# facebookresearch/sylph-few-shot-detection

Measured on AMD Instinct MI355X. Metric: query images/sec, R50-FPN 5-way 5-shot 800x1333 (whole job), higher is better.
Workload: dtype bf16

## Files before the change

### sylph-few-shot-detection_amd/csrc/conv_hpipe.hip

```cpp
#include <stdlib.h>

#include "common.h"

#ifndef SYLPH_ABLATE
#undef HP_NOWAITV
#undef HP_NOLDS
#undef HP_NOLOAD
#undef HP_NOEPI
#undef HP_TIMING
#endif

namespace sylph {

typedef __attribute__((address_space(3))) void* lds_ptr_t;
typedef const __attribute__((address_space(1))) void* gbl_ptr_t;

namespace {
constexpr int PNT = 512;
constexpr int BSTAGE = 256 * 64;
constexpr int NSTAGE = 4;
constexpr int HPROWS = 256;
constexpr int HBUF = 2 * HPROWS * 64;
constexpr int HALO_OFF = NSTAGE * BSTAGE;
constexpr int COEF_OFF = HALO_OFF + 2 * HBUF;
constexpr int COEF_MAX_CIN = 512;
constexpr int LDS_BYTES = COEF_OFF + 2 * COEF_MAX_CIN * 8;
constexpr int SCP = 256 + 4;
static_assert(64 * SCP * 4 <= LDS_BYTES, "epilogue tile must fit");

constexpr int NPIECE = 2 * HPROWS / 128;
constexpr int nload(int t) { return ((t % 9 + 9) % 9) < NPIECE ? 3 : 2; }

#define HP_SCHED_FENCE __builtin_amdgcn_sched_barrier(0)
#define HP_BAR()                                   \
  do {                                             \
    asm volatile("" ::: "memory");                 \
    HP_SCHED_FENCE;                                \
    __builtin_amdgcn_s_barrier();                  \
    HP_SCHED_FENCE;                                \
    asm volatile("" ::: "memory");                 \
  } while (0)
#ifdef HP_NOWAITV
#define HP_WAITV(N) asm volatile("" ::: "memory")
#else
#define HP_WAITV(N) asm volatile("s_waitcnt vmcnt(%0)" ::"n"(N) : "memory")
#endif
#define HP_WAITL() asm volatile("s_waitcnt lgkmcnt(0)" ::: "memory")
}

template <bool GNIN>
__global__ __launch_bounds__(PNT, 1) void conv_hpipe_kernel(const ConvArgs a) {
  typedef bf16_t T;
  extern __shared__ __attribute__((aligned(16))) char smem[];

  const int L = blockIdx.x;
  const int xcd = L & 7, q0 = L >> 3;
  const int chunk = (a.n_mtiles + 7) >> 3;
  const int m_local = q0 / a.n_ntiles;
  const int nt = q0 - m_local * a.n_ntiles;
  const int mt = xcd * chunk + m_local;
  if (m_local >= chunk || mt >= a.n_mtiles) return;
#ifdef HP_TIMING
  const unsigned long long hp_t0 = __builtin_readcyclecounter();
  unsigned long long hp_t1 = 0, hp_t2 = 0;
#endif

  const int tid = threadIdx.x, lane = tid & 63;
  const int wave = __builtin_amdgcn_readfirstlane(tid >> 6);
  const int wm = wave >> 2, wn = wave & 3;
  const int l31 = lane & 31, lh = lane >> 5;

  int2 tl0 = a.tiles[2 * mt], tl1 = a.tiles[2 * mt + 1];
  const int rot_key = (int)((unsigned)tl0.x >> 20);
  tl0.x &= 0xfffff;
  const SegDesc sd0 = a.segs[tl0.x], sd1 = a.segs[tl1.x];

  const T* __restrict__ in = reinterpret_cast<const T*>(a.in);
  const T* __restrict__ wt = reinterpret_cast<const T*>(a.wt);
  const T* __restrict__ zero = reinterpret_cast<const T*>(a.zeros);
  const int Cin = a.Cin;
  const int ncc = Cin >> 5;
  const int goff = a.group_cout > 0 ? ((nt * 256) / a.group_cout) * a.group_in_off : 0;
  const int c0 = (rot_key + nt) % ncc;

  const int r4 = tid >> 2, s4 = tid & 3;
  const char* hptr[NPIECE];
  unsigned hmask = 0, hcs = 0;
#pragma unroll
  for (int g = 0; g < NPIECE; ++g) {
    const bool p1 = g >= NPIECE / 2;
    const SegDesc& sd = p1 ? sd1 : sd0;
    const int ty = p1 ? tl1.y : tl0.y;
    const int h = g * 128 + r4 - (p1 ? HPROWS : 0);
    const int PW = sd.pw, HP = sd.hpitch, HR = (sd.ph + 2) * HP;
    const int hy = (int)(((unsigned)h * sd.inv_hw2) >> 16), hx = h - hy * HP;
    const int iy = (ty >> 16) - 1 + hy, ix = (ty & 0xffff) - 1 + hx;
    const bool ok = h < HR && hx < PW + 2 && (unsigned)iy < (unsigned)sd.in_H && (unsigned)ix < (unsigned)sd.in_W;
    const int cs = s4 ^ (((hy * PW + hx) >> 2) & 3);
    hcs |= (unsigned)cs << (2 * g);
    hptr[g] = ok ? reinterpret_cast<const char*>(in + ((size_t)(sd.in_row0 + iy * sd.in_W + ix) * a.in_ld + cs * 8 + goff + c0 * 32))
                 : reinterpret_cast<const char*>(zero + s4 * 8);
    hmask |= (ok ? 1u : 0u) << g;
  }
  const char* const wtile = reinterpret_cast<const char*>(wt) + (size_t)nt * ncc * 9 * BSTAGE;
  const unsigned wvo = (unsigned)tid * 16u;
  bool loads_on = true;
  auto issue_halo = [&](int g, int buf) {
    if (!loads_on) return;
    {
    char* d = smem + HALO_OFF + buf * HBUF + g * 8192 + wave * 1024;
    __builtin_amdgcn_global_load_lds((gbl_ptr_t)hptr[g], (lds_ptr_t)d, 16, 0, 0);
    }
  };
  auto advance_halo = [&](int cc_next) {
    const int step = (c0 + cc_next == ncc) ? (32 - Cin) * 2 : 64;
#pragma unroll
    for (int g = 0; g < NPIECE; ++g) hptr[g] += ((hmask >> g) & 1u) ? step : 0;
  };
  auto issue_w = [&](int stage, int j, int blk) {
    if (!loads_on) return;
    {
    char* d = smem + stage * BSTAGE + j * 8192 + wave * 1024;
    const char* src = wtile + (size_t)blk * BSTAGE + j * 8192 + wvo;
    __builtin_amdgcn_global_load_lds((gbl_ptr_t)src, (lds_ptr_t)d, 16, 0, 0);
    }
  };
  auto rot = [&](int cc) { const int c = c0 + cc; return c >= ncc ? c - ncc : c; };

  constexpr bool gn_in = GNIN;
  const bool gn_relu = a.gn_relu != 0;
  typedef unsigned u32x4 __attribute__((ext_vector_type(4)));
  typedef float f32x4v __attribute__((ext_vector_type(4)));
  const unsigned lds0 = (unsigned)(size_t)(__attribute__((address_space(3))) char*)smem;
  u32x4 gx;
  f32x4v gc0, gc1, gc2, gc3;
  auto gn_addr = [&](int g, int cc_of_piece) { return lds0 + HALO_OFF + (cc_of_piece & 1) * HBUF + g * 8192 + tid * 16; };
  auto gn_read = [&](int g, int cc_of_piece) {
    const unsigned d = gn_addr(g, cc_of_piece);
    const int ch = rot(cc_of_piece) * 32 + (int)((hcs >> (2 * g)) & 3u) * 8;
    const unsigned cf = lds0 + COEF_OFF + ((g >= NPIECE / 2 ? Cin : 0) + ch) * 8;
    asm volatile("ds_read_b128 %0, %1" : "=v"(gx) : "v"(d));
    asm volatile("ds_read_b128 %0, %1" : "=v"(gc0) : "v"(cf));
    asm volatile("ds_read_b128 %0, %1 offset:16" : "=v"(gc1) : "v"(cf));
    asm volatile("ds_read_b128 %0, %1 offset:32" : "=v"(gc2) : "v"(cf));
    asm volatile("ds_read_b128 %0, %1 offset:48" : "=v"(gc3) : "v"(cf));
  };
  auto gn_finish = [&](int g, int cc_of_piece) {
    asm volatile("s_waitcnt lgkmcnt(0)" : "+v"(gx), "+v"(gc0), "+v"(gc1), "+v"(gc2), "+v"(gc3));
    const unsigned live = ((hmask >> g) & 1u) ? 0xffffffffu : 0u;
    const f32x4v cs[4] = {gc0, gc1, gc2, gc3};
    typedef float f32x2v __attribute__((ext_vector_type(2)));
    typedef short s16x2v __attribute__((ext_vector_type(2)));
    typedef __attribute__((ext_vector_type(2))) __bf16 bf16x2;
    u32x4 y;
#pragma unroll
    for (int e = 0; e < 4; ++e) {
      const f32x2v xv = {__uint_as_float(gx[e] << 16), __uint_as_float(gx[e] & 0xffff0000u)};
      const f32x2v av = {cs[e][0], cs[e][1]}, bv = {cs[e][2], cs[e][3]};
      const f32x2v r = __builtin_elementwise_fma(xv, av, bv);
      bf16x2 pk;
      pk[0] = (bf16_t)r[0]; pk[1] = (bf16_t)r[1];
      unsigned u = __builtin_bit_cast(unsigned, pk);
      if (gn_relu) {
        const s16x2v z = {0, 0};
        u = __builtin_bit_cast(unsigned, __builtin_elementwise_max(__builtin_bit_cast(s16x2v, u), z));
      }
      y[e] = u & live;
    }
    asm volatile("ds_write_b128 %0, %1" ::"v"(gn_addr(g, cc_of_piece)), "v"(y) : "memory");
  };
  auto gn_piece = [&](int g, int cc_of_piece) { gn_read(g, cc_of_piece); gn_finish(g, cc_of_piece); };

  const SegDesc& sdm = wm ? sd1 : sd0;
  const int PWm = sdm.pw, HW2m = sdm.hpitch;
  int a0[4];
#pragma unroll
  for (int i = 0; i < 4; ++i) {
    const int m = i * 32 + l31;
    const int my = (int)(((unsigned)m * sdm.inv_pw) >> 16);
    a0[i] = (wm * HPROWS + my * HW2m + (m - my * PWm)) * 64;
  }
  int offB[2];
#pragma unroll
  for (int ks = 0; ks < 2; ++ks) offB[ks] = (wn * 64 + l31) * 64 + (((ks * 2 + lh) ^ ((l31 >> 2) & 3)) << 4);

  f32x16 acc[4][2];
#pragma unroll
  for (int i = 0; i < 4; ++i)
#pragma unroll
    for (int j = 0; j < 2; ++j)
#pragma unroll
      for (int r = 0; r < 16; ++r) acc[i][j][r] = 0.f;
  bf16x8 fa[2][4], fb[2][2];

  auto ldfrag = [&](int cc, int t) {
    const int kh = t / 3, kw = t - 3 * kh;
    const char* bs = smem + ((cc + t) & 3) * BSTAGE;
    const char* hs = smem + HALO_OFF + (cc & 1) * HBUF + (kh * HW2m + kw) * 64;
    const int f = ((l31 + kh * PWm + kw) >> 2) & 3;
#ifdef HP_NOLDS
    if (cc + t > 0) return;
#endif
#pragma unroll
    for (int ks = 0; ks < 2; ++ks) {
      const int so = ((ks * 2 + lh) ^ f) << 4;
#pragma unroll
      for (int j = 0; j < 2; ++j) fb[ks][j] = *reinterpret_cast<const bf16x8*>(bs + offB[ks] + j * 2048);
#pragma unroll
      for (int i = 0; i < 4; ++i) fa[ks][i] = *reinterpret_cast<const bf16x8*>(hs + a0[i] + so);
    }
  };

  auto issue_next = [&](int cc, int t) {
    const int t3 = (t + 3) % 9, cc3 = cc + (t + 3) / 9;
    const int blk = cc3 < ncc ? rot(cc3) * 9 + t3 : 0;
    const int st3 = (cc + t + 3) & 3;
    if (t == 0 && cc + 1 < ncc) advance_halo(cc + 1);
    if (t < NPIECE) issue_halo(t, (cc + 1) & 1);
    issue_w(st3, 0, blk);
    issue_w(st3, 1, blk);
  };
  auto mma = [&](int cc, int t) {
    __builtin_amdgcn_s_setprio(1);
    const bool xf = gn_in && t >= 3 && t < 3 + NPIECE;
    if (xf) {
      gn_read(t - 3, cc + 1);
      HP_SCHED_FENCE;
    }
    int n = 0;
#pragma unroll
    for (int ks = 0; ks < 2; ++ks)
#pragma unroll
      for (int i = 0; i < 4; ++i)
#pragma unroll
        for (int j = 0; j < 2; ++j) {
          acc[i][j] = __builtin_amdgcn_mfma_f32_32x32x16_bf16(fb[ks][j], fa[ks][i], acc[i][j], 0, 0, 0);
          if (xf && n == 3) {
            HP_SCHED_FENCE;
            gn_finish(t - 3, cc + 1);
          }
          ++n;
        }
    if (xf) {
#pragma unroll
      for (int k = 0; k < 12; ++k) {
        __builtin_amdgcn_sched_group_barrier(0x008, 1, 0);
        __builtin_amdgcn_sched_group_barrier(0x002, 4, 0);
      }
    }
    __builtin_amdgcn_s_setprio(0);
  };

  auto frags_ready = [&]() {
    asm volatile("" ::"v"(fa[0][0]), "v"(fa[0][1]), "v"(fa[0][2]), "v"(fa[0][3]), "v"(fa[1][0]), "v"(fa[1][1]), "v"(fa[1][2]),
                 "v"(fa[1][3]), "v"(fb[0][0]), "v"(fb[0][1]), "v"(fb[1][0]), "v"(fb[1][1]));
  };

#pragma unroll
  for (int g = 0; g < NPIECE; ++g) issue_halo(g, 0);
#pragma unroll
  for (int t = 0; t < 3; ++t) {
    issue_w(t, 0, c0 * 9 + t);
    issue_w(t, 1, c0 * 9 + t);
  }
#ifdef HP_NOLOAD
  issue_w(3, 0, c0 * 9 + 3); issue_w(3, 1, c0 * 9 + 3);
  for (int g = 0; g < NPIECE; ++g) issue_halo(g, 1);
  HP_WAITV(0);
  loads_on = false;
#endif
  if (gn_in) {
    for (int idx = tid; idx < Cin; idx += PNT) {
      const int pch = idx >= Cin / 2 ? 1 : 0, ch = (idx - pch * (Cin / 2)) * 2;
      const int seg = pch ? tl1.x : tl0.x;
      const float2 c0v = a.gn_coef[(size_t)seg * a.in_ld + goff + ch], c1v = a.gn_coef[(size_t)seg * a.in_ld + goff + ch + 1];
      *reinterpret_cast<float4*>(smem + COEF_OFF + (pch * Cin + ch) * 8) = make_float4(c0v.x, c1v.x, c0v.y, c1v.y);
    }
  }
  HP_WAITV(4);
  if (gn_in) {
    HP_WAITL();
    HP_BAR();
#pragma unroll
    for (int g = 0; g < NPIECE; ++g) gn_piece(g, 0);
    HP_WAITL();
  }
  HP_BAR();
#ifdef HP_TIMING
  hp_t1 = __builtin_readcyclecounter();
#endif

#define HP_PHASE0(t)                      \
  ldfrag(cc, t);                          \
  HP_SCHED_FENCE;                         \
  issue_next(cc, t);                      \
  HP_WAITL();                             \
  if (GNIN) frags_ready();                \
  HP_BAR();                               \
  mma(cc, t);                             \
  HP_WAITV(nload((t) - 1) + nload(t));    \
  HP_BAR();
#define HP_PHASE1(t)                      \
  ldfrag(cc, t);                          \
  HP_SCHED_FENCE;                         \
  issue_next(cc, t);                      \
  HP_WAITV(nload((t) - 1) + nload(t));    \
  HP_WAITL();                             \
  if (GNIN) frags_ready();                \
  HP_BAR();                               \
  mma(cc, t);                             \
  HP_BAR();

  if (wm == 0) {
    for (int cc = 0; cc < ncc; ++cc) {
      HP_PHASE0(0) HP_PHASE0(1) HP_PHASE0(2) HP_PHASE0(3) HP_PHASE0(4) HP_PHASE0(5) HP_PHASE0(6) HP_PHASE0(7) HP_PHASE0(8)
    }
    HP_BAR();
  } else {
    HP_BAR();
    for (int cc = 0; cc < ncc; ++cc) {
      HP_PHASE1(0) HP_PHASE1(1) HP_PHASE1(2) HP_PHASE1(3) HP_PHASE1(4) HP_PHASE1(5) HP_PHASE1(6) HP_PHASE1(7) HP_PHASE1(8)
    }
  }
  asm volatile("s_waitcnt vmcnt(0)" ::: "memory");
  __syncthreads();
#ifdef HP_TIMING
  hp_t2 = __builtin_readcyclecounter();
#endif

  float* const sC = reinterpret_cast<float*>(smem);
  bf16_t* __restrict__ out = reinterpret_cast<bf16_t*>(a.out);
  const int c8 = tid & 31, rr = tid >> 5;
  const int n0 = nt * 256 + c8 * 8;
  float sc[8], sh[8];
#pragma unroll
  for (int h = 0; h < 2; ++h) {
    const float4 s4v = a.scale ? reinterpret_cast<const float4*>(a.scale + n0)[h] : make_float4(1.f, 1.f, 1.f, 1.f);
    const float4 b4v = a.shift ? reinterpret_cast<const float4*>(a.shift + n0)[h] : make_float4(0.f, 0.f, 0.f, 0.f);
    sc[4 * h] = s4v.x; sc[4 * h + 1] = s4v.y; sc[4 * h + 2] = s4v.z; sc[4 * h + 3] = s4v.w;
    sh[4 * h] = b4v.x; sh[4 * h + 1] = b4v.y; sh[4 * h + 2] = b4v.z; sh[4 * h + 3] = b4v.w;
  }
  const bool relu = a.relu_nch > 0;
#pragma unroll
  for (int pp = 0; pp < 2; ++pp) {
    const SegDesc& sp = pp ? sd1 : sd0;
    const int ty = pp ? tl1.y : tl0.y;
    const int oy0 = ty >> 16, ox0 = ty & 0xffff;
    const int PW = sp.pw, NPOS = sp.ph * sp.pw;
    bf16_t* __restrict__ outn = out + (size_t)sp.out_row0 * a.out_ld + n0;
    float gn_n = 0.f, gn_s1 = 0.f, gn_s2 = 0.f;
    const float gn_pv = sh[0];
#pragma unroll
    for (int hp = 0; hp < 2; ++hp) {
      if (pp + hp > 0) lds_barrier();
      if (wm == pp) {
#pragma unroll
        for (int ii = 0; ii < 2; ++ii)
#pragma unroll
          for (int j = 0; j < 2; ++j)
#pragma unroll
            for (int g = 0; g < 4; ++g) {
              const f32x16& c = acc[2 * hp + ii][j];
              *reinterpret_cast<float4*>(sC + (ii * 32 + l31) * SCP + wn * 64 + j * 32 + 8 * g + 4 * lh) =
                  make_float4(c[4 * g], c[4 * g + 1], c[4 * g + 2], c[4 * g + 3]);
            }
      }
      lds_barrier();
#pragma unroll
      for (int it = 0; it < 4; ++it) {
        const int rl = rr + 16 * it;
        const int m = hp * 64 + rl;
        const int my = (int)(((unsigned)m * sp.inv_pw) >> 16);
        const int oy = oy0 + my, ox = ox0 + (m - my * PW);
        if (m < NPOS && oy < sp.out_H && ox < sp.out_W) {
          float v[8];
          const float4 lo = *reinterpret_cast<const float4*>(sC + rl * SCP + c8 * 8);
          const float4 hi = *reinterpret_cast<const float4*>(sC + rl * SCP + c8 * 8 + 4);
          v[0] = lo.x; v[1] = lo.y; v[2] = lo.z; v[3] = lo.w; v[4] = hi.x; v[5] = hi.y; v[6] = hi.z; v[7] = hi.w;
#pragma unroll
          for (int e = 0; e < 8; ++e) v[e] = v[e] * sc[e] + sh[e];
          if (relu) {
#pragma unroll
            for (int e = 0; e < 8; ++e) v[e] = v[e] > 0.f ? v[e] : 0.f;
          }
          if (a.gn_partial) {
#pragma unroll
            for (int e = 0; e < 8; ++e) { const float d = v[e] - gn_pv; gn_s1 += d; gn_s2 = fmaf(d, d, gn_s2); }
            gn_n += 8.f;
          }
#ifndef HP_NOEPI
          store8<bf16_t>(outn + (size_t)(oy * sp.out_W + ox) * a.out_ld, v);
#else
          if (v[0] == 1234.5f) store8<bf16_t>(outn + (size_t)(oy * sp.out_W + ox) * a.out_ld, v);
#endif
        }
      }
    }
    if (a.gn_partial) {
      gn_n += __shfl_xor(gn_n, 32);
      gn_s1 += __shfl_xor(gn_s1, 32);
      gn_s2 += __shfl_xor(gn_s2, 32);
      lds_barrier();
      float* red = sC;
      if (lane < 32) {
        red[(wave * 32 + c8) * 3 + 0] = gn_n;
        red[(wave * 32 + c8) * 3 + 1] = gn_s1;
        red[(wave * 32 + c8) * 3 + 2] = gn_s2;
      }
      lds_barrier();
      if (tid < 32) {
        float N = 0.f, S1 = 0.f, S2 = 0.f;
#pragma unroll
        for (int w = 0; w < 8; ++w) {
          N += red[(w * 32 + c8) * 3 + 0]; S1 += red[(w * 32 + c8) * 3 + 1]; S2 += red[(w * 32 + c8) * 3 + 2];
        }
        const float inv_n = N > 0.f ? 1.f / N : 0.f;
        const float m2 = S2 - S1 * S1 * inv_n;
        float* gp = a.gn_partial + ((size_t)(2 * mt + pp) * (a.Cout >> 3) + (n0 >> 3)) * 3;
        gp[0] = N; gp[1] = gn_pv + S1 * inv_n; gp[2] = m2 > 0.f ? m2 : 0.f;
      }
    }
  }
#ifdef HP_TIMING
  if (L >= 2048 && L < 2048 + 64 && (tid == 0 || tid == 256)) {
    const unsigned long long t3 = __builtin_readcyclecounter();
    printf("blk %d row %d: prologue %llu  K loop %llu  epilogue %llu cycles\n", L, tid >> 8, hp_t1 - hp_t0, hp_t2 - hp_t1, t3 - hp_t2);
  }
#endif
}

__global__ void hpipe_pack_weights_kernel(const bf16_t* __restrict__ w, bf16_t* __restrict__ out, int Cout, int Cin) {
  const size_t i = (size_t)blockIdx.x * blockDim.x + threadIdx.x;
  const size_t nchunks = (size_t)Cout * 9 * Cin / 8;
  if (i >= nchunks) return;
  const int ncc = Cin >> 5;
  const int s = (int)(i & 3), r = (int)((i >> 2) & 255);
  const size_t blk = i >> 10;
  const int t = (int)(blk % 9), c = (int)((blk / 9) % ncc), nt = (int)(blk / (9 * (size_t)ncc));
  const int chunk = s ^ ((r >> 2) & 3);
  const uint4 v = *reinterpret_cast<const uint4*>(w + ((size_t)(nt * 256 + r) * 9 + t) * Cin + c * 32 + chunk * 8);
  *reinterpret_cast<uint4*>(out + i * 8) = v;
}

int launch_hpipe_pack_weights(const void* w, void* out, int Cout, int Cin, hipStream_t s) {
  const size_t nchunks = (size_t)Cout * 9 * Cin / 8;
  hipLaunchKernelGGL(hpipe_pack_weights_kernel, dim3((unsigned)((nchunks + 255) / 256)), dim3(256), 0, s, (const bf16_t*)w, (bf16_t*)out, Cout, Cin);
  return (int)hipGetLastError();
}

bool conv_hpipe_ok(DType dt, bool out_f32, const ConvArgs& a) {
  if (a.gn_coef && (a.Cin > COEF_MAX_CIN || a.group_cout > 0)) return false;
  return dt == DT_BF16 && !out_f32 && !a.stem && !a.in2 && a.res_mode == 0 && a.mul_nch == 0 && a.KH == 3 && a.KW == 3 &&
         a.stride == 1 && a.pad == 1 && (a.relu_nch == 0 || a.relu_nch >= a.Cout) && a.Cout % 256 == 0 && a.Cin % 32 == 0 &&
         a.Cin >= 32 && a.ss_padded_host && (a.out_ld & 7) == 0 && a.zeros != nullptr;
}

#ifdef SYLPH_ABLATE
int launch_conv_hq(const ConvArgs& a, hipStream_t s);
#endif

int launch_conv_hpipe(const ConvArgs& a, hipStream_t s) {
#if defined(SYLPH_ABLATE) && defined(SYLPH_HQ_PROBE)
  static const int hq = SYLPH_AB_ENV("SYLPH_CONV_HQ", 0);
  if (hq) return launch_conv_hq(a, s);
#endif
  static bool attr_set = false;
  if (!attr_set) {
    if (hipFuncSetAttribute((const void*)conv_hpipe_kernel<false>, hipFuncAttributeMaxDynamicSharedMemorySize, LDS_BYTES) != hipSuccess) return -7;
    if (hipFuncSetAttribute((const void*)conv_hpipe_kernel<true>, hipFuncAttributeMaxDynamicSharedMemorySize, LDS_BYTES) != hipSuccess) return -7;
    attr_set = true;
  }
  const int chunk = (a.n_mtiles + 7) / 8;
  const int grid = 8 * chunk * a.n_ntiles;
  if (a.gn_coef) hipLaunchKernelGGL(conv_hpipe_kernel<true>, dim3(grid), dim3(PNT), LDS_BYTES, s, a);
  else hipLaunchKernelGGL(conv_hpipe_kernel<false>, dim3(grid), dim3(PNT), LDS_BYTES, s, a);
  return (int)hipGetLastError();
}

}
```

Before: 2245.

## Switch hpipe conv to 16x16x32 MFMA tiles with new LDS swizzle

Replaces the 32x32x16 bf16 MFMA tiling (4x2 accumulators, two k-substeps) with 16x16x32 MFMA over an 8x4 accumulator grid, and changes the LDS XOR swizzle for halo, weights and the packing kernel to match the new fragment read pattern. The GN input path now converts to bf16 with a vector convert and applies a branch-free max against a floor value instead of a conditional ReLU. The scheduling barriers and epilogue stores are reworked for the new accumulator shape. This trades the larger MFMA for more instructions, each with a shorter latency, and an altered bank-conflict profile.

Measured after the change: 2347 (median of 6 runs). 1.05x the previous value.

```diff
diff --git a/sylph-few-shot-detection_amd/csrc/conv_hpipe.hip b/sylph-few-shot-detection_amd/csrc/conv_hpipe.hip
--- a/sylph-few-shot-detection_amd/csrc/conv_hpipe.hip
+++ b/sylph-few-shot-detection_amd/csrc/conv_hpipe.hip
@@ -68,7 +68,7 @@
   const int tid = threadIdx.x, lane = tid & 63;
   const int wave = __builtin_amdgcn_readfirstlane(tid >> 6);
   const int wm = wave >> 2, wn = wave & 3;
-  const int l31 = lane & 31, lh = lane >> 5;
+  const int l15 = lane & 15, lq = lane >> 4;
 
   int2 tl0 = a.tiles[2 * mt], tl1 = a.tiles[2 * mt + 1];
   const int rot_key = (int)((unsigned)tl0.x >> 20);
@@ -96,7 +96,7 @@
     const int hy = (int)(((unsigned)h * sd.inv_hw2) >> 16), hx = h - hy * HP;
     const int iy = (ty >> 16) - 1 + hy, ix = (ty & 0xffff) - 1 + hx;
     const bool ok = h < HR && hx < PW + 2 && (unsigned)iy < (unsigned)sd.in_H && (unsigned)ix < (unsigned)sd.in_W;
-    const int cs = s4 ^ (((hy * PW + hx) >> 2) & 3);
+    const int cs = s4 ^ ((((hy * PW + hx) >> 2) & 1) << 1);
     hcs |= (unsigned)cs << (2 * g);
     hptr[g] = ok ? reinterpret_cast<const char*>(in + ((size_t)(sd.in_row0 + iy * sd.in_W + ix) * a.in_ld + cs * 8 + goff + c0 * 32))
                  : reinterpret_cast<const char*>(zero + s4 * 8);
@@ -128,7 +128,7 @@
   auto rot = [&](int cc) { const int c = c0 + cc; return c >= ncc ? c - ncc : c; };
 
   constexpr bool gn_in = GNIN;
-  const bool gn_relu = a.gn_relu != 0;
+  const short gn_floor = a.gn_relu != 0 ? (short)0 : (short)-32768;
   typedef unsigned u32x4 __attribute__((ext_vector_type(4)));
   typedef float f32x4v __attribute__((ext_vector_type(4)));
   const unsigned lds0 = (unsigned)(size_t)(__attribute__((address_space(3))) char*)smem;
@@ -158,13 +158,9 @@
       const f32x2v xv = {__uint_as_float(gx[e] << 16), __uint_as_float(gx[e] & 0xffff0000u)};
       const f32x2v av = {cs[e][0], cs[e][1]}, bv = {cs[e][2], cs[e][3]};
       const f32x2v r = __builtin_elementwise_fma(xv, av, bv);
-      bf16x2 pk;
-      pk[0] = (bf16_t)r[0]; pk[1] = (bf16_t)r[1];
-      unsigned u = __builtin_bit_cast(unsigned, pk);
-      if (gn_relu) {
-        const s16x2v z = {0, 0};
-        u = __builtin_bit_cast(unsigned, __builtin_elementwise_max(__builtin_bit_cast(s16x2v, u), z));
-      }
+      const bf16x2 pk = __builtin_convertvector(r, bf16x2);
+      const s16x2v fl = {gn_floor, gn_floor};
+      const unsigned u = __builtin_bit_cast(unsigned, __builtin_elementwise_max(__builtin_bit_cast(s16x2v, pk), fl));
       y[e] = u & live;
     }
     asm volatile("ds_write_b128 %0, %1" ::"v"(gn_addr(g, cc_of_piece)), "v"(y) : "memory");
@@ -173,42 +169,38 @@
 
   const SegDesc& sdm = wm ? sd1 : sd0;
   const int PWm = sdm.pw, HW2m = sdm.hpitch;
-  int a0[4];
-#pragma unroll
-  for (int i = 0; i < 4; ++i) {
-    const int m = i * 32 + l31;
+  int a0[8];
+#pragma unroll
+  for (int i = 0; i < 8; ++i) {
+    const int m = i * 16 + l15;
     const int my = (int)(((unsigned)m * sdm.inv_pw) >> 16);
     a0[i] = (wm * HPROWS + my * HW2m + (m - my * PWm)) * 64;
   }
-  int offB[2];
-#pragma unroll
-  for (int ks = 0; ks < 2; ++ks) offB[ks] = (wn * 64 + l31) * 64 + (((ks * 2 + lh) ^ ((l31 >> 2) & 3)) << 4);
-
-  f32x16 acc[4][2];
-#pragma unroll
-  for (int i = 0; i < 4; ++i)
-#pragma unroll
-    for (int j = 0; j < 2; ++j)
-#pragma unroll
-      for (int r = 0; r < 16; ++r) acc[i][j][r] = 0.f;
-  bf16x8 fa[2][4], fb[2][2];
+  const int offB = (wn * 64 + l15) * 64 + ((lq ^ (((l15 >> 2) & 1) << 1)) << 4);
+
+  f32x4 acc[8][4];
+#pragma unroll
+  for (int i = 0; i < 8; ++i)
+#pragma unroll
+    for (int j = 0; j < 4; ++j)
+#pragma unroll
+      for (int r = 0; r < 4; ++r) acc[i][j][r] = 0.f;
+  bf16x8 fa[8], fb[4];
 
   auto ldfrag = [&](int cc, int t) {
     const int kh = t / 3, kw = t - 3 * kh;
     const char* bs = smem + ((cc + t) & 3) * BSTAGE;
     const char* hs = smem + HALO_OFF + (cc & 1) * HBUF + (kh * HW2m + kw) * 64;
-    const int f = ((l31 + kh * PWm + kw) >> 2) & 3;
+    int key = l15;
+    asm volatile("" : "+v"(key));
+    const int so = (lq ^ ((((key + kh * PWm + kw) >> 2) & 1) << 1)) << 4;
 #ifdef HP_NOLDS
     if (cc + t > 0) return;
 #endif
 #pragma unroll
-    for (int ks = 0; ks < 2; ++ks) {
-      const int so = ((ks * 2 + lh) ^ f) << 4;
-#pragma unroll
-      for (int j = 0; j < 2; ++j) fb[ks][j] = *reinterpret_cast<const bf16x8*>(bs + offB[ks] + j * 2048);
-#pragma unroll
-      for (int i = 0; i < 4; ++i) fa[ks][i] = *reinterpret_cast<const bf16x8*>(hs + a0[i] + so);
-    }
+    for (int j = 0; j < 4; ++j) fb[j] = *reinterpret_cast<const bf16x8*>(bs + offB + j * 1024);
+#pragma unroll
+    for (int i = 0; i < 8; ++i) fa[i] = *reinterpret_cast<const bf16x8*>(hs + a0[i] + so);
   };
 
   auto issue_next = [&](int cc, int t) {
@@ -229,31 +221,29 @@
     }
     int n = 0;
 #pragma unroll
-    for (int ks = 0; ks < 2; ++ks)
-#pragma unroll
-      for (int i = 0; i < 4; ++i)
-#pragma unroll
-        for (int j = 0; j < 2; ++j) {
-          acc[i][j] = __builtin_amdgcn_mfma_f32_32x32x16_bf16(fb[ks][j], fa[ks][i], acc[i][j], 0, 0, 0);
-          if (xf && n == 3) {
-            HP_SCHED_FENCE;
-            gn_finish(t - 3, cc + 1);
-          }
-          ++n;
+    for (int i = 0; i < 8; ++i)
+#pragma unroll
+      for (int j = 0; j < 4; ++j) {
+        acc[i][j] = __builtin_amdgcn_mfma_f32_16x16x32_bf16(fb[j], fa[i], acc[i][j], 0, 0, 0);
+        if (xf && n == 7) {
+          HP_SCHED_FENCE;
+          gn_finish(t - 3, cc + 1);
         }
+        ++n;
+      }
     if (xf) {
 #pragma unroll
-      for (int k = 0; k < 12; ++k) {
+      for (int k = 0; k < 16; ++k) {
         __builtin_amdgcn_sched_group_barrier(0x008, 1, 0);
-        __builtin_amdgcn_sched_group_barrier(0x002, 4, 0);
+        __builtin_amdgcn_sched_group_barrier(0x002, 2, 0);
       }
     }
     __builtin_amdgcn_s_setprio(0);
   };
 
   auto frags_ready = [&]() {
-    asm volatile("" ::"v"(fa[0][0]), "v"(fa[0][1]), "v"(fa[0][2]), "v"(fa[0][3]), "v"(fa[1][0]), "v"(fa[1][1]), "v"(fa[1][2]),
-                 "v"(fa[1][3]), "v"(fb[0][0]), "v"(fb[0][1]), "v"(fb[1][0]), "v"(fb[1][1]));
+    asm volatile("" ::"v"(fa[0]), "v"(fa[1]), "v"(fa[2]), "v"(fa[3]), "v"(fa[4]), "v"(fa[5]), "v"(fa[6]), "v"(fa[7]), "v"(fb[0]),
+                 "v"(fb[1]), "v"(fb[2]), "v"(fb[3]));
   };
 
 #pragma unroll
@@ -355,15 +345,12 @@
       if (pp + hp > 0) lds_barrier();
       if (wm == pp) {
 #pragma unroll
-        for (int ii = 0; ii < 2; ++ii)
-#pragma unroll
-          for (int j = 0; j < 2; ++j)
-#pragma unroll
-            for (int g = 0; g < 4; ++g) {
-              const f32x16& c = acc[2 * hp + ii][j];
-              *reinterpret_cast<float4*>(sC + (ii * 32 + l31) * SCP + wn * 64 + j * 32 + 8 * g + 4 * lh) =
-                  make_float4(c[4 * g], c[4 * g + 1], c[4 * g + 2], c[4 * g + 3]);
-            }
+        for (int ii = 0; ii < 4; ++ii)
+#pragma unroll
+          for (int j = 0; j < 4; ++j) {
+            const f32x4& c = acc[4 * hp + ii][j];
+            *reinterpret_cast<float4*>(sC + (ii * 16 + l15) * SCP + wn * 64 + j * 16 + 4 * lq) = make_float4(c[0], c[1], c[2], c[3]);
+          }
       }
       lds_barrier();
 #pragma unroll
@@ -437,7 +424,7 @@
   const int s = (int)(i & 3), r = (int)((i >> 2) & 255);
   const size_t blk = i >> 10;
   const int t = (int)(blk % 9), c = (int)((blk / 9) % ncc), nt = (int)(blk / (9 * (size_t)ncc));
-  const int chunk = s ^ ((r >> 2) & 3);
+  const int chunk = s ^ (((r >> 2) & 1) << 1);
   const uint4 v = *reinterpret_cast<const uint4*>(w + ((size_t)(nt * 256 + r) * 9 + t) * Cin + c * 32 + chunk * 8);
   *reinterpret_cast<uint4*>(out + i * 8) = v;
 }
```
